# gmlwns2000/sharkshark-4k

Hardware: AMD Instinct MI355X
Metric: upscaled frames/sec at 720p->1440p x2 (whole job) (higher is better)
Workload: dtype f16; 1 GPU; RealESRGAN RRDBNet x2 (23 blocks) 720p->1440p fp16 [BASELINE configs[2]]; io=uint8 NHWC resident in HBM

## Files before the change

sharkshark-4k_amd/csrc/common.h:

```cpp
#pragma once
#include <hip/hip_runtime.h>
#include <hip/hip_fp16.h>
#include <algorithm>
#include <cstdint>
#include <cstdio>
#include <cstdlib>
#include <cstring>
#include <map>
#include <tuple>
#include <set>
#include <string>
#include <vector>
#include <stdexcept>
#include "../../include/ss4k.h"
#ifdef SS4K_DEV
#include "../../include/ss4k_dev.h"
#endif

namespace ss4k {

void set_error(const char* fmt, ...);

struct Error : std::runtime_error {
  int code;
// ... 111 lines not shown
    return lane_stream_;
  }
  static hipEvent_t untimed_event(hipEvent_t& e) {
    if (!e && hipEventCreateWithFlags(&e, hipEventDisableTiming) != hipSuccess) throw ss4k::Error(SS4K_EHIP, "hipEventCreateWithFlags failed");
    return e;
  }
  hipEvent_t lane_fork() { return untimed_event(fork_event); }
  hipEvent_t lane_done() { return untimed_event(done_event); }
  std::set<hipStream_t> lane_checked;
  std::vector<hipStream_t> lane_parked;
  int lane_replaced = 0;
  void lane_check(hipStream_t caller);
#ifdef SS4K_DEV
  int dev_handicap_lane = 0; unsigned dev_handicap_ticks = 0;
  int64_t dev_lane_forks = 0, dev_lane_joins = 0, dev_lane_spins = 0;
  int dev_drop_join = 0;
#endif
  std::vector<ss4k::ProfEvent> prof_sections;
  double prof_section_ms = 0;
  ss4k::ProfEvent prof_get_events() {
    ss4k::ProfEvent pe{};
    if (!prof_pool.empty()) { pe = prof_pool.back(); prof_pool.pop_back(); pe.flops = 0; pe.kind = 0; pe.family = nullptr; return pe; }
    if (hipEventCreate(&pe.a) != hipSuccess || hipEventCreate(&pe.b) != hipSuccess) throw ss4k::Error(SS4K_EHIP, "hipEventCreate failed");
    return pe;
  }
  ss4k::ProfEvent prof_begin(hipStream_t st, int kind) {
    ss4k::ProfEvent pe{};
    if (!prof) return pe;
    pe = prof_get_events(); pe.kind = kind;
    if (hipEventRecord(pe.a, st) != hipSuccess) throw ss4k::Error(SS4K_EHIP, "hipEventRecord failed");
    return pe;
  }
  void prof_end(ss4k::ProfEvent pe, hipStream_t st, double flops) {
    if (!pe.a) return;
    if (hipEventRecord(pe.b, st) != hipSuccess) throw ss4k::Error(SS4K_EHIP, "hipEventRecord failed");
    pe.flops = flops; pe.family = prof_family; prof_family = nullptr; prof_events.push_back(pe);
  }
  const char* zero_page() {
    auto& b = scratch["zero_page"];
    if (!b.ptr) { b.ensure(256); (void)hipMemset(b.ptr, 0, 256); }
    return b.as<char>();
  }
  struct CvAreaTab { std::vector<char> host; ss4k::DevBuf dev; hipEvent_t uploaded = nullptr; int oh = 0, ow = 0; size_t xe = 0, xo = 0, ye = 0, yo = 0; };
  std::map<std::tuple<int, int, double, double>, CvAreaTab> cv_area;
  ss4k::DevBuf& buf(const std::string& name, size_t bytes) {
    auto& b = scratch[name];
    b.ensure(bytes);
#ifdef SS4K_DEV
    b.transient = true;
#endif
    return b;
  }
};

namespace ss4k {

struct ProfScope {
  ss4k_ctx* ctx; hipStream_t st; ProfEvent pe; bool open;
  ProfScope(ss4k_ctx* c, hipStream_t s, int kind) : ctx(c), st(s), pe(c->prof_begin(s, kind)), open(true) {}
  void done(double flops) { if (open) { open = false; ctx->prof_end(pe, st, flops); } }
  ~ProfScope() { if (open && pe.a) ctx->prof_pool.push_back(pe); }
  ProfScope(const ProfScope&) = delete; ProfScope& operator=(const ProfScope&) = delete;
};

enum Act { ACT_NONE = 0, ACT_LRELU = 1, ACT_PRELU = 2, ACT_RELU6 = 3 };
enum Epi {
  EPI_NHWC = 0,
  EPI_NHWC_SUB2 = 1,
  EPI_NHWC_PS2 = 2,
  EPI_NCHW_F32 = 3
};

struct ConvArgs {
  const char* in0; size_t in0_plane_bytes; int in0_plane0, nchunks0;
  const char* in1; size_t in1_plane_bytes; int in1_plane0, nchunks1;
  const char* zero_page;
  int N, H, W;
  int n0;
  int job_n;
  float grid_share;
  int mb_override;
  int wide_rl;
  int wide;
  int no_band;
  int ups2;
  int ups_presum;
  const void* wpk;
  const void* w16;
  const float* bias;
  const float* prelu;
  int prelu_le1;
  int act; float slope;
  float alpha, gamma;
  const char* res1; size_t r1_plane_bytes; int r1_plane0;
  const char* res2; size_t r2_plane_bytes; int r2_plane0;
  int bsvd_resid;
  int epi;
  char* out; size_t out_plane_bytes; int out_plane0;
  int cout_real, cout_pad;
  int tiles_x, tiles_y;
  int reverse;
  double flops;
  int dbg;
  unsigned long long* dbg_buf;
};
inline double conv_plane_span_f16(const ConvArgs& a) { return (double)std::max(a.n0 + a.N, a.job_n) * a.H * a.W * 32.0; }
enum { DBG_NO_STORE = 1, DBG_NO_MMA = 2, DBG_NO_TILE_DMA = 4, DBG_NO_W_DMA = 8, DBG_NO_EPILOGUE = 16, DBG_STAMP = 32 };

void launch_conv3x3(ss4k_ctx* ctx, const ConvArgs& a, int dtype, hipStream_t st);
struct PairArgs {
  const char* in; size_t in_plane_bytes; int in_plane0, planes_a;
  const char* wA; const float* biasA;
  const char* wB; const float* biasB;
  const char* res; size_t res_plane_bytes; int res_plane0;
  const char* zero_page;
  unsigned long long* dbg_buf;
  char* out; size_t out_plane_bytes; int out_plane0;
  int epi;
  int cout_real;
  int n0, N, H, W, bands;
  float grid_share;
  double flops;
};
inline bool conv3x3_pair_eligible(int planes_a, int cout_pad_a, int nchunks_b, int cout_pad_b) {
  return (planes_a == 1 || planes_a == 2) && cout_pad_a == 32 && nchunks_b == 2 && cout_pad_b == 32;
}
void launch_conv3x3_pair(ss4k_ctx* ctx, const PairArgs& a, hipStream_t st);

struct DenseArgs {
  const char* in0; size_t in0_plane_bytes; int in0_plane0, nchunks0;
  const char* in1; size_t in1_plane_bytes; int in1_plane0, nchunks1;
  const char* w1; const float* bias1;
  const char* w2; const float* bias2;
  float slope;
  char* out1; size_t out1_plane_bytes; int out1_plane0;
  char* out2; size_t out2_plane_bytes; int out2_plane0;
  const char* zero_page;
  int n0, N, H, W, tiles_x, tiles_y;
  float grid_share;
  int reverse;
  double flops;
  unsigned long long* dbg_buf;
};
inline bool conv3x3_dense2_eligible(int nchunks_a, int cout_pad_a, int nchunks_b, int cout_pad_b) {
  return cout_pad_a == 32 && cout_pad_b == 32 && nchunks_b == nchunks_a + 2 && nchunks_a >= 2 && nchunks_a % 2 == 0;
}
struct ConvArgs;
bool conv3x3_wide_eligible(const ConvArgs& a, int dtype);
void launch_conv3x3_wide(ss4k_ctx* ctx, const ConvArgs& a, hipStream_t st);
void launch_conv3x3_dense2(ss4k_ctx* ctx, const DenseArgs& a, hipStream_t st);
bool conv3x3_w16_eligible(const ConvArgs& a, int dtype);
void launch_conv3x3_w16(ss4k_ctx* ctx, const ConvArgs& a, hipStream_t st);
bool conv3x3_w16n_eligible(const ConvArgs& a, int dtype);
void launch_conv3x3_w16n(ss4k_ctx* ctx, const ConvArgs& a, hipStream_t st);

inline int conv_cw(int) { return 16; }
inline int cout_pad_of(int cout) { return cout <= 32 ? 32 : (cout + 63) / 64 * 64; }
inline int conv_rec_bytes(int dtype) { return dtype == SS4K_F16 ? 32 : 64; }

struct PackSpec {
  int dtype;
  int cout_real, cin_total;
  std::vector<int> cin_map;
  int nchunks0, nchunks1;
  int ps2;
};
// ... 13 lines not shown
```

sharkshark-4k_amd/csrc/conv_tile.h:

```cpp
#pragma once
#include "common.h"

namespace ss4k {

typedef float f32x16 __attribute__((ext_vector_type(16)));
typedef _Float16 f16x8 __attribute__((ext_vector_type(8)));

constexpr int TW = 32, IN_W = TW + 2;
constexpr uint32_t OOB = 0xFFFFFFFFu;
template <typename T> struct Tr;
template <> struct Tr<__half> { static constexpr int E = 8, KS = 1; };
template <> struct Tr<float> { static constexpr int E = 4, KS = 2; };
constexpr int CW = 16;

template <typename T, int MB, int NW> struct Geo {
  static constexpr int KS = Tr<T>::KS, SPR = 2 * KS, REC = 16 * SPR;
  static constexpr int TH = NW * MB, IN_H = TH + 2, IN_PIX = IN_W * IN_H;
  static constexpr int TILE_SLOTS = IN_PIX * SPR;
  static constexpr int TILE_DMA = (TILE_SLOTS + 63) / 64;
  static constexpr int DMA_PER_WAVE = (TILE_DMA + NW - 1) / NW;
};
template <typename T, int NB, int MB, int NW> constexpr size_t lds_bytes() {
  return (size_t)(2 * Geo<T, MB, NW>::TILE_SLOTS + 2 * 9 * Tr<T>::KS * NB * 64) * 16 + NB * 32 * 2 * 4;
}
template <typename T, int NB, int MB, int NW> constexpr int wgs_per_cu() {
  return NW == 8 ? 1 : (lds_bytes<T, NB, MB, NW>() <= 53 * 1024 ? 3 : lds_bytes<T, NB, MB, NW>() <= 80 * 1024 ? 2 : 1);
}

__device__ __forceinline__ void dma16(const void* gsrc, uint32_t lds_addr_wave_uniform) {
  uint32_t keep;
  asm volatile("s_mov_b32 %0, m0\n\ts_mov_b32 m0, %2\n\ts_nop 0\n\tglobal_load_lds_dwordx4 %1, off\n\ts_mov_b32 m0, %0"
               : "=&s"(keep)
               : "v"(gsrc), "s"(lds_addr_wave_uniform)
               : "memory");
}
__device__ __forceinline__ void dma_wait() { asm volatile("s_waitcnt vmcnt(0)" ::: "memory"); }

template <typename T> __device__ __forceinline__ void load16(const char* p, float* v);
template <> __device__ __forceinline__ void load16<__half>(const char* p, float* v) {
  const uint4 a = *reinterpret_cast<const uint4*>(p), b = *reinterpret_cast<const uint4*>(p + 16);
  const __half* ha = reinterpret_cast<const __half*>(&a);
  const __half* hb = reinterpret_cast<const __half*>(&b);
#pragma unroll
  for (int i = 0; i < 8; ++i) { v[i] = __half2float(ha[i]); v[8 + i] = __half2float(hb[i]); }
}
template <> __device__ __forceinline__ void load16<float>(const char* p, float* v) {
#pragma unroll
  for (int q = 0; q < 4; ++q) {
    const float4 a = *reinterpret_cast<const float4*>(p + 16 * q);
    v[4 * q] = a.x; v[4 * q + 1] = a.y; v[4 * q + 2] = a.z; v[4 * q + 3] = a.w;
  }
}
template <typename T> __device__ __forceinline__ void store16(char* p, const float* v);
template <> __device__ __forceinline__ void store16<__half>(char* p, const float* v) {
  uint4 a, b;
  __half* ha = reinterpret_cast<__half*>(&a);
  __half* hb = reinterpret_cast<__half*>(&b);
#pragma unroll
  for (int i = 0; i < 8; ++i) { ha[i] = __float2half(v[i]); hb[i] = __float2half(v[8 + i]); }
  *reinterpret_cast<uint4*>(p) = a;
  *reinterpret_cast<uint4*>(p + 16) = b;
}
template <> __device__ __forceinline__ void store16<float>(char* p, const float* v) {
#pragma unroll
  for (int q = 0; q < 4; ++q)
    *reinterpret_cast<float4*>(p + 16 * q) = make_float4(v[4 * q], v[4 * q + 1], v[4 * q + 2], v[4 * q + 3]);
}

template <typename T> __device__ __forceinline__ void load8(const char* p, float* v);
template <> __device__ __forceinline__ void load8<__half>(const char* p, float* v) {
  const uint4 a = *reinterpret_cast<const uint4*>(p);
  const __half* ha = reinterpret_cast<const __half*>(&a);
#pragma unroll
  for (int i = 0; i < 8; ++i) v[i] = __half2float(ha[i]);
}
template <> __device__ __forceinline__ void load8<float>(const char* p, float* v) {
#pragma unroll
  for (int q = 0; q < 2; ++q) {
    const float4 a = *reinterpret_cast<const float4*>(p + 16 * q);
    v[4 * q] = a.x; v[4 * q + 1] = a.y; v[4 * q + 2] = a.z; v[4 * q + 3] = a.w;
  }
}
typedef unsigned int u32x4 __attribute__((ext_vector_type(4)));
template <typename T> __device__ __forceinline__ void store8(char* p, const float* v);
template <> __device__ __forceinline__ void store8<__half>(char* p, const float* v) {
  uint4 a;
  __half* ha = reinterpret_cast<__half*>(&a);
#pragma unroll
  for (int i = 0; i < 8; ++i) ha[i] = __float2half(v[i]);
  __builtin_nontemporal_store(*reinterpret_cast<u32x4*>(&a), reinterpret_cast<u32x4*>(p));
}
template <> __device__ __forceinline__ void store8<float>(char* p, const float* v) {
#pragma unroll
  for (int q = 0; q < 2; ++q) {
    const float4 f = make_float4(v[4 * q], v[4 * q + 1], v[4 * q + 2], v[4 * q + 3]);
    __builtin_nontemporal_store(*reinterpret_cast<const u32x4*>(&f), reinterpret_cast<u32x4*>(p + 16 * q));
  }
}

__device__ __forceinline__ void lds_barrier() {
  __builtin_amdgcn_fence(__ATOMIC_RELEASE, "workgroup", "local");
  __builtin_amdgcn_s_barrier();
  __builtin_amdgcn_fence(__ATOMIC_ACQUIRE, "workgroup", "local");
}

template <typename T>
__device__ __forceinline__ f32x16 mma(const uint4& w, const uint4& x, f32x16 acc) {
  if constexpr (sizeof(T) == 2) {
    return __builtin_amdgcn_mfma_f32_32x32x16_f16(*reinterpret_cast<const f16x8*>(&w),
                                                  *reinterpret_cast<const f16x8*>(&x), acc, 0, 0, 0);
  } else {
    const float* wf = reinterpret_cast<const float*>(&w);
    const float* xf = reinterpret_cast<const float*>(&x);
#pragma unroll
    for (int j = 0; j < 4; ++j) acc = __builtin_amdgcn_mfma_f32_32x32x2f32(wf[j], xf[j], acc, 0, 0, 0);
    return acc;
// ... 5 lines not shown
```

sharkshark-4k_amd/csrc/conv_w16.hip:

```cpp
#include "common.h"
#include <cmath>
#include "conv_tile.h"
#include <type_traits>
#include <cstdio>
#include <cstdlib>
#include <vector>

namespace ss4k {
namespace w16 {

typedef float f32x4 __attribute__((ext_vector_type(4)));

constexpr int NW = 4, MB = 8, TH = 16;
constexpr int XH = TH + 2, XW = TW + 2;
constexpr int REC = 32;
constexpr int ROWX = XW * REC;
constexpr int XT_SLOTS = XH * XW * 2;
constexpr int XT_BYTES = XT_SLOTS * 16;
constexpr int XT_DMA = (XT_SLOTS + 63) / 64;
constexpr int DMA_PER_WAVE = (XT_DMA + NW - 1) / NW;
constexpr int WP = 12 * 1024, NWS = 3;
constexpr int NDMA = DMA_PER_WAVE + 3;
constexpr int W_OFF = 2 * XT_BYTES, B_OFF = W_OFF + NWS * WP;
constexpr size_t LDS_BYTES = B_OFF + 2 * 64 * 4;
static_assert(2 * LDS_BYTES <= 160 * 1024, "two workgroups per CU");

__device__ __forceinline__ f32x4 mma16(const uint4& w, const uint4& x, f32x4 acc) {
  return __builtin_amdgcn_mfma_f32_16x16x32_f16(__builtin_bit_cast(f16x8, w), __builtin_bit_cast(f16x8, x), acc, 0, 0, 0);
}

#ifdef SS4K_DEV
template <bool STAMP = false, bool RL = false, bool GEN = false>
#else
template <bool STAMP = false, bool RL = false>
#endif
__global__ __launch_bounds__(64 * NW, 2) void conv3x3_w16_kernel(const ConvArgs a) {
#ifndef SS4K_DEV
  constexpr bool GEN = false;
#endif
  extern __shared__ __attribute__((aligned(16))) char smem[];
  const uint32_t lds0 = (uint32_t)(size_t)(__attribute__((address_space(3))) char*)smem;
  const int tid = threadIdx.x, lane = tid & 63;
  const int wave = __builtin_amdgcn_readfirstlane(tid >> 6);
  const int n16 = lane & 15, kg = lane >> 4;
  const int rgp = wave & 1, jw = wave >> 1;
  const int grp = blockIdx.y;
  const int K = a.nchunks0 + a.nchunks1, NP = K >> 1;
  const int ntiles = a.N * a.tiles_y * a.tiles_x;
  const char* wbase = reinterpret_cast<const char*>(a.w16) + (size_t)grp * NP * (3 * WP);

  unsigned long long ph[6] = {0, 0, 0, 0, 0, 0}, tlast = 0, rt0 = 0, ct0 = 0;
  if constexpr (STAMP) { rt0 = __builtin_amdgcn_s_memrealtime(); ct0 = __builtin_amdgcn_s_memtime(); tlast = ct0; }
  auto stamp = [&](int k) {
    if constexpr (STAMP) {
      unsigned long long t;
      __builtin_amdgcn_sched_barrier(0);
      asm volatile("s_memtime %0\n\ts_waitcnt lgkmcnt(0)" : "=s"(t)::"memory");
      __builtin_amdgcn_sched_barrier(0);
      ph[k] += t - tlast;
      tlast = t;
    }
  };
  const bool banded = (gridDim.x % 8 == 0) && ntiles >= (int)gridDim.x && !a.no_band;
  const int tpx = (ntiles + 7) / 8;
  auto tile_of = [&](int k) -> int {
    if (!banded) {
      const int t = blockIdx.x + k * gridDim.x;
      return t < ntiles ? (a.reverse ? ntiles - 1 - t : t) : -1;
    }
    const int base = (blockIdx.x & 7) * tpx, len = min(tpx, ntiles - base);
    const int j = (blockIdx.x >> 3) + k * (gridDim.x >> 3);
    return j < len ? base + (a.reverse ? len - 1 - j : j) : -1;
  };
  int rdA[2], rdX[2];
#pragma unroll
  for (int hn = 0; hn < 2; ++hn) {
    rdA[hn] = (((rgp * MB) * XW + 16 * hn + n16 + (kg >> 1)) * 2 + (kg & 1)) * 16;
    rdX[hn] = (((rgp * MB) * XW + 16 * hn + n16 + 2) * 2 + (kg & 1)) * 16 + (kg >> 1) * XT_BYTES;
  }

  auto setup_tile = [&](int tile, int& n, int& y0, int& x0) {
    const int tx = tile % a.tiles_x, tyn = tile / a.tiles_x;
    const int ty = tyn % a.tiles_y;
    n = a.n0 + tyn / a.tiles_y; y0 = ty * TH; x0 = tx * TW;
  };
  auto tile_src = [&](int k, int n, int y0, int x0) -> uint32_t {
    const int s = k * 64 + lane;
    const int p = s >> 1, gq = s & 1;
    const int row = p / XW, x = p - row * XW;
    const int iy = y0 - 1 + row, ix = x0 - 1 + x;
    const bool ok = s < XT_SLOTS && iy >= 0 && iy < a.H && ix >= 0 && ix < a.W;
    return ok ? ((uint32_t)(n * a.H + iy) * (uint32_t)a.W + (uint32_t)ix) * REC + (uint32_t)(gq * 16) : OOB;
  };
  auto plane_of = [&](int c) {
    return (c < a.nchunks0) ? a.in0 + (size_t)(a.in0_plane0 + c) * a.in0_plane_bytes
                            : a.in1 + (size_t)(a.in1_plane0 + c - a.nchunks0) * a.in1_plane_bytes;
  };
  const char* pf_plane = nullptr; const char* pf_w = nullptr; int pf_buf = 0, pf_slot = 0, pf_n = 0, pf_y0 = 0, pf_x0 = 0; bool pf_tile = false, pf_wt = false;
  auto dma_op = [&](int idx) {
    if (idx < DMA_PER_WAVE) {
      const int k = wave + NW * idx;
      if (pf_tile && k < XT_DMA) {
        const uint32_t so = tile_src(k, pf_n, pf_y0, pf_x0);
        const char* src = so != OOB ? pf_plane + so : a.zero_page + (lane & 3) * 16;
        const uint32_t dst = __builtin_amdgcn_readfirstlane(lds0 + pf_buf * XT_BYTES + k * 1024);
        if (k * 64 + lane < XT_SLOTS) dma16(src, dst);
      }
    } else if (idx < NDMA) {
      const int k = wave + NW * (idx - DMA_PER_WAVE);
      if (pf_wt) dma16(pf_w + k * 1024 + lane * 16, __builtin_amdgcn_readfirstlane(lds0 + W_OFF + pf_slot * WP + k * 1024));
    }
  };
  auto slot_inc = [](int s) { return s == NWS - 1 ? 0 : s + 1; };
  auto lane_now = [] {
    unsigned z = 0;
    asm volatile("" : "+v"(z));
    return (int)__builtin_amdgcn_mbcnt_hi(~0u, __builtin_amdgcn_mbcnt_lo(~0u, z));
  };

  float* epi_lds = reinterpret_cast<float*>(smem + B_OFF);
  if (tid < 64) {
    const int mbk = tid >> 4, q = (tid >> 2) & 3, i = tid & 3;
    const int vb = grp * 64 + 32 * (mbk >> 1) + 16 * (q >> 1) + 8 * (q & 1) + 4 * (mbk & 1) + i;
    epi_lds[tid] = vb < a.cout_pad ? a.bias[vb] : 0.f;
    const int v = grp * 64 + tid;
    epi_lds[64 + tid] = a.act == ACT_PRELU ? (v < a.cout_pad ? a.prelu[v] : 1.f) : (a.act == ACT_LRELU ? a.slope : (a.act == ACT_RELU6 ? 0.f : 1.f));
  }

  int kt = 0;
  int tile = tile_of(0);
  if (tile < 0) return;
  int n, y0, x0;
  setup_tile(tile, n, y0, x0);
  pf_n = n; pf_y0 = y0; pf_x0 = x0;
  int ws = 0;
  pf_tile = true; pf_plane = plane_of(0); pf_buf = 0; pf_wt = true; pf_w = wbase; pf_slot = 0;
#pragma unroll
  for (int i = 0; i < NDMA; ++i) dma_op(i);
  pf_tile = false; pf_w = wbase + WP; pf_slot = 1;
#pragma unroll
  for (int i = DMA_PER_WAVE; i < NDMA; ++i) dma_op(i);
  dma_wait();
  __syncthreads();
  const int lane16 = lane * 16;
  const int wsub = lane16 + jw * 2048;
  uint4 wf[3][2];
#pragma unroll
  for (int dy = 0; dy < 3; ++dy)
#pragma unroll
    for (int e = 0; e < 2; ++e) wf[dy][e] = *reinterpret_cast<const uint4*>(smem + W_OFF + wsub + (dy * 4 + e) * 1024);

  while (true) {
    f32x4 acc[MB][2][2];
    f32x4 bias4[2];
    {
      const float4* bp = reinterpret_cast<const float4*>(smem + B_OFF + (lane_now() >> 4) * 16 + jw * 128);
      const float4 b0 = bp[0], b1 = bp[4];
      bias4[0] = f32x4{b0.x, b0.y, b0.z, b0.w}; bias4[1] = f32x4{b1.x, b1.y, b1.z, b1.w};
    }
    const int cur_n = n, cur_y0 = y0, cur_x0 = x0;
    const int next_tile = tile_of(kt + 1);
    stamp(0);

    auto period = [&](const int q, auto FIRSTP) {
      const bool last_q = q + 1 == NP;
      auto phase = [&](auto PH, auto FIRST) {
        constexpr int ph = decltype(PH)::value;
        constexpr bool first = decltype(FIRST)::value;
        const int lp2 = 3 * q + ph + 2;
        if (lp2 < 3 * NP) { pf_wt = true; pf_w = wbase + (size_t)lp2 * WP; }
        else if (next_tile >= 0) { pf_wt = true; pf_w = wbase + (size_t)(lp2 - 3 * NP) * WP; }
        else pf_wt = false;
        pf_slot = ws == 0 ? NWS - 1 : ws - 1;
        if constexpr (ph == 0) { pf_tile = true; pf_plane = plane_of(2 * q + 1); pf_buf = 1; }
        else if constexpr (ph == 1) { pf_tile = false; }
        else {
          pf_buf = 0;
          if (!last_q) { pf_tile = true; pf_plane = plane_of(2 * q + 2); }
          else if (next_tile >= 0) { setup_tile(next_tile, n, y0, x0); pf_n = n; pf_y0 = y0; pf_x0 = x0; pf_tile = true; pf_plane = plane_of(0); }
          else pf_tile = false;
        }
        const bool more = !(last_q && ph == 2) || next_tile >= 0;
        const char* tb = smem + (ph == 2 ? XT_BYTES : 0);
        const int* rd = ph == 1 ? rdX : rdA;
        const char* wbn = smem + W_OFF + slot_inc(ws) * WP + wsub;
        uint4 bf[3][2];
        auto bf_load = [&](int t, int hn) { return *reinterpret_cast<const uint4*>(tb + rd[hn] + t * ROWX); };
        bool rl_on = false;
        uint32_t idw[2] = {0u, 0u};
        if constexpr (RL && ph != 1) {
          rl_on = q == jw;
          const int rg = (lane & 15) >> 2, i = lane & 3;
          const bool hit = kg >= 2 && (kg & 1) == (rg & 1) && (rg >> 1) == (ph >> 1);
          const uint32_t hv = hit ? (uint32_t)__half_as_ushort(__float2half(1.f / a.alpha)) << (16 * (i & 1)) : 0u;
          idw[0] = (i >> 1) == 0 ? hv : 0u; idw[1] = (i >> 1) == 1 ? hv : 0u;
        }
#pragma unroll
        for (int t = 0; t < 3; ++t) { bf[t][0] = bf_load(t, 0); bf[t][1] = bf_load(t, 1); }
        int m = 0;
        __builtin_amdgcn_sched_barrier(0);
        __builtin_amdgcn_s_setprio(1);
#pragma unroll
        for (int ir = 0; ir < MB + 2; ++ir) {
#pragma unroll
          for (int dy = 0; dy < 3; ++dy) {
            const int r = ir - dy;
            if (r >= 0 && r < MB) {
#pragma unroll
              for (int hn = 0; hn < 2; ++hn) {
#pragma unroll
                for (int e = 0; e < 2; ++e) acc[r][hn][e] = mma16(wf[dy][e], bf[ir % 3][hn], (first && dy == 0) ? bias4[e] : acc[r][hn][e]);
                if constexpr (RL && ph != 1) {
                  if (dy == 1 && rl_on) {
#pragma unroll
                    for (int e = 0; e < 2; ++e)
                      acc[r][hn][e] = mma16(e == 0 ? make_uint4(idw[0], idw[1], 0u, 0u) : make_uint4(0u, 0u, idw[0], idw[1]), bf[ir % 3][hn], acc[r][hn][e]);
                  }
                }
                const int sl = (m & 1) && m < 10 ? m >> 1 : (m == 13 || m == 17 || m == 21) ? DMA_PER_WAVE + (m - 13) / 4 : -1;
                if (sl >= 0) {
                  __builtin_amdgcn_sched_barrier(0);
                  dma_op(sl);
                  __builtin_amdgcn_sched_barrier(0);
                }
                ++m;
              }
            }
          }
          __builtin_amdgcn_sched_barrier(0);
          if (ir + 3 < MB + 2) { bf[ir % 3][0] = bf_load(ir + 3, 0); bf[ir % 3][1] = bf_load(ir + 3, 1); }
          if (more && ir >= MB - 1) {
            const int dy = ir - (MB - 1);
#pragma unroll
            for (int e = 0; e < 2; ++e) wf[dy][e] = *reinterpret_cast<const uint4*>(wbn + (dy * 4 + e) * 1024);
          }
          __builtin_amdgcn_sched_barrier(0);
        }
        __builtin_amdgcn_s_setprio(0);
        stamp(ph == 1 ? 2 : 1);
        if (more) { dma_wait(); stamp(3); __syncthreads(); stamp(4); }
        ws = slot_inc(ws);
      };
      phase(std::integral_constant<int, 0>{}, FIRSTP);
      phase(std::integral_constant<int, 1>{}, std::false_type{});
      phase(std::integral_constant<int, 2>{}, std::false_type{});
    };
    period(0, std::true_type{});
#pragma unroll 1
    for (int q = 1; q < NP; ++q) period(q, std::false_type{});

    {
      const float alpha = a.alpha, gamma = a.gamma;
      const int le = lane_now();
      const int kge = le >> 4, n16e = le & 15;
      auto load_slopes = [&](float* s) {
        const float4* sp = reinterpret_cast<const float4*>(epi_lds + 64 + 32 * jw + 8 * kge);
        const float4 s0 = sp[0], s1 = sp[1];
        s[0] = s0.x; s[1] = s0.y; s[2] = s0.z; s[3] = s0.w;
        s[4] = s1.x; s[5] = s1.y; s[6] = s1.z; s[7] = s1.w;
      };
      const int opl = grp * 4 + 2 * jw + (kge >> 1);
      const size_t sub = (size_t)(kge & 1) * 16;
      const char* r1p = (a.res1 && !RL) ? a.res1 + (size_t)(a.r1_plane0 + opl) * a.r1_plane_bytes + sub : nullptr;
// ... 281 lines not shown
```

sharkshark-4k_amd/csrc/models.cpp:

```cpp
#include "models.h"
#include <algorithm>
#include <cmath>
#include <cstdlib>
#include <cstring>

namespace ss4k {

static size_t esz(int dtype) { return dtype == SS4K_F16 ? 2 : 4; }
static int pad16(int c) { return (c + 15) / 16 * 16; }


static std::vector<std::pair<int, int>> bsvd_denblock_shapes(const int* chns, int in_ch, int out_ch, int interm) {
  const int c0 = chns[0], c1 = chns[1], c2 = chns[2];
  return {{interm, in_ch}, {c0, interm}, {c1, c0}, {c1, c1}, {c1, c1}, {c2, c1}, {c2, c2}, {c2, c2},
          {c2, c2}, {c2, c2}, {c1 * 4, c2}, {c1, c1}, {c1, c1}, {c0 * 4, c1}, {c0, c0}, {out_ch, c0}};
}

static void validate_desc(const ss4k_model_desc& d);

size_t model_param_count(const ss4k_model_desc& d) {
  try { validate_desc(d); } catch (const Error&) { return 0; }
  switch (d.kind) {
    case SS4K_FSRCNN:
      return 56 * 25 + 56 + 56 + 12 * 56 + 12 + 12 + 4 * (12 * 12 * 9 + 12 + 12) + 56 * 12 + 56 + 56 + 56 * 81 + 1;
// ... 80 lines not shown
  if (a) upload(L.prelu, p.prelu.data(), p.prelu.size() * 4);
  if (use_w16 && use_wide && desc.dtype == SS4K_F16 && p.nb == 2 && p.cout_pad % 64 == 0 && (s.nchunks0 + s.nchunks1) % 2 == 0 && !s.ps2) {
    const std::vector<uint8_t> w6 = pack_conv3x3_w16(s, w, p.cout_pad);
    upload(L.w16, w6.data(), w6.size());
    weight_bytes += w6.size();
  }
  if (use_w16 && desc.dtype == SS4K_F16 && cout <= 4 && (s.nchunks0 + s.nchunks1) % 2 == 0 && !s.ps2) {
    const std::vector<uint8_t> w6 = pack_conv3x3_w16n(s, w);
    upload(L.w16, w6.data(), w6.size());
    weight_bytes += w6.size();
  }
  L.has_prelu = a != nullptr;
  if (a) { L.prelu_le1 = true; for (int c = 0; c < cout; ++c) L.prelu_le1 = L.prelu_le1 && a[c] <= 1.f; }
  L.cout_real = cout; L.cout_pad = p.cout_pad; L.nchunks0 = s.nchunks0; L.nchunks1 = s.nchunks1;
  L.cin_real = 0;
  for (int c : s.cin_map) L.cin_real += c >= 0;
  weight_bytes += p.w.size() + p.bias.size() * 4;
  layers.push_back(std::move(L));
  return (int)layers.size() - 1;
}

PackSpec Model::spec_plain(int cin_real, int ps2) const {
  PackSpec s{}; s.ps2 = ps2; s.nchunks0 = planes_for(cin_real); s.nchunks1 = 0;
  s.cin_map.assign((size_t)s.nchunks0 * cw(), -1);
  for (int j = 0; j < cin_real; ++j) s.cin_map[j] = j;
  return s;
}
PackSpec Model::spec_concat(int c0, int c1) const {
  PackSpec s{}; s.nchunks0 = planes_for(c0); s.nchunks1 = planes_for(c1);
  s.cin_map.assign((size_t)(s.nchunks0 + s.nchunks1) * cw(), -1);
  for (int j = 0; j < c0; ++j) s.cin_map[j] = j;
  for (int j = 0; j < c1; ++j) s.cin_map[(size_t)s.nchunks0 * cw() + j] = c0 + j;
  return s;
}
PackSpec Model::spec_masked(int c) const {
  PackSpec s{}; const int first = (c / 4) / cw();
  s.nchunks0 = planes_for(c) - first; s.nchunks1 = 0;
  s.cin_map.assign((size_t)s.nchunks0 * cw(), -1);
  for (int j = 0; j < s.nchunks0 * cw(); ++j) {
    const int ch = first * cw() + j;
    if (ch >= c / 4 && ch < c) s.cin_map[j] = ch;
  }
  return s;
}

PackSpec Model::spec_shifted(int c) const {
  PackSpec s{}; const int lead = shifted_planes(c);
  s.nchunks0 = lead; s.nchunks1 = planes_for(c) - lead;
  s.cin_map.assign((size_t)planes_for(c) * cw(), -1);
  for (int j = 0; j < c; ++j) s.cin_map[j] = j;
  return s;
}

void Model::build(const float* w, size_t n) {
  validate_desc(desc);
  const int fl = desc.flags;
  SS4K_REQUIRE((fl & ~SS4K_MODEL_FLAGS_ALL) == 0, "desc.flags: unknown SS4K_MODEL_* bit (bits 8, 64, 128, 2048 and 16384 were retired with ABI 3)");
  SS4K_REQUIRE(!((fl & SS4K_MODEL_ONE_CHAIN) && (fl & SS4K_MODEL_TWO_CHAINS)), "desc.flags: ONE_CHAIN and TWO_CHAINS exclude each other");
  SS4K_REQUIRE(!((fl & SS4K_MODEL_TILE_ROWS_16) && (fl & SS4K_MODEL_TILE_ROWS_20)), "desc.flags: TILE_ROWS_16 and TILE_ROWS_20 exclude each other");
  if (fl & SS4K_MODEL_FS_EXACT) fs_exact = true;
  if (fl & SS4K_MODEL_ONE_CHAIN) lanes_mode = 1;
  if (fl & SS4K_MODEL_TWO_CHAINS) lanes_mode = 2;
  if (fl & SS4K_MODEL_TILE_ROWS_16) mb_override = 4;
  if (fl & SS4K_MODEL_TILE_ROWS_20) mb_override = 5;
  if (fl & SS4K_MODEL_NO_PAIR) use_pair = false;
  if (fl & SS4K_MODEL_NO_DENSE) dense_mode = 1;
  if (fl & SS4K_MODEL_HR_F32) hr_f32 = true;
  if (fl & SS4K_MODEL_NO_WIDE) use_wide = false;
  if (fl & SS4K_MODEL_NO_UPS_PRESUM) ups_presum = false;
  if (fl & SS4K_MODEL_NO_W16) use_w16 = false;
  if (!(fl & (SS4K_MODEL_ONE_CHAIN | SS4K_MODEL_TWO_CHAINS)))
    if (const char* e = std::getenv("SS4K_LANES")) lanes_mode = std::max(0, std::min(2, std::atoi(e)));
  if (const char* e = std::getenv("SS4K_FS_EXACT")) fs_exact = fs_exact || e[0] == '1';
#ifdef SS4K_DEV
  if (const char* e = std::getenv("SS4K_NO_FLIP")) flip_walk = !(e[0] == '1');
  if (const char* e = std::getenv("SS4K_SUBBATCH")) sub_batch = std::atoi(e);
  if (const char* e = std::getenv("SS4K_MB")) mb_override = std::atoi(e);
  if (const char* e = std::getenv("SS4K_DENSE_MASK")) dense_mask = std::atoi(e);
  if (const char* e = std::getenv("SS4K_UPS_PRESUM")) ups_presum = e[0] == '1';
  if (const char* e = std::getenv("SS4K_NO_RL")) no_rl = e[0] == '1';
  if (const char* e = std::getenv("SS4K_WIDE_RL")) wide_rl = e[0] == '1';
  if (const char* e = std::getenv("SS4K_WIDE")) use_wide = e[0] == '1';
  if (const char* e = std::getenv("SS4K_W16")) use_w16 = e[0] == '1';
  if (const char* e = std::getenv("SS4K_DENSE_MODE")) dense_mode = std::atoi(e);
  if (const char* e = std::getenv("SS4K_LANE_GRID")) lane_grid_share = (float)std::atof(e);
  if (const char* e = std::getenv("SS4K_FAIL_AT_CONV")) fail_at_conv = std::atoi(e);
#endif
  SS4K_REQUIRE(n == model_param_count(desc), "weight blob size does not match the model description");
  ParamCursor pc{w, n};
  if (desc.kind == SS4K_FSRCNN) {
    weight_bytes = fsrcnn_pack_weights(pc, fs_exact, fs_blob, fsw);
  } else if (desc.kind == SS4K_RRDBNET) {
    const int nf = desc.num_feat, g = desc.num_grow_ch;
    const int cin0 = 3 * (desc.scale == 2 ? 4 : desc.scale == 1 ? 16 : 1);
    add_conv(pc, nf, cin0, spec_plain(cin0), false);
    for (int b = 0; b < desc.num_block; ++b)
      for (int r = 0; r < 3; ++r)
        for (int c = 0; c < 5; ++c) {
          const int co = c < 4 ? g : nf;
          add_conv(pc, co, nf + c * g, c == 0 ? spec_plain(nf) : spec_concat(nf, c * g), false);
        }
    for (int i = 0; i < 4; ++i) add_conv(pc, nf, nf, spec_plain(nf), false);
    add_conv(pc, 3, nf, spec_plain(nf), false);
  } else if (desc.kind == SS4K_SRVGG) {
    const int nf = desc.num_feat;
    add_conv(pc, nf, 3, spec_plain(3), true);
    for (int i = 0; i < desc.num_block; ++i) add_conv(pc, nf, nf, spec_plain(nf), true);
    add_conv(pc, 3 * desc.scale * desc.scale, nf, spec_plain(nf), false);
  } else {
    for (int blk = 0; blk < 2; ++blk) {
      const int ci = blk == 0 ? 4 : desc.bsvd_mid_ch, co = blk == 0 ? desc.bsvd_mid_ch : 3;
      auto shapes = bsvd_denblock_shapes(desc.bsvd_chns, ci, co, desc.bsvd_interm_ch);
      for (size_t i = 0; i < shapes.size(); ++i) {
        const int cout = shapes[i].first, cin = shapes[i].second;
        const bool masked = (i == 3 || i == 4 || i == 6 || i == 7 || i == 8 || i == 9 || i == 11 || i == 12);
        const bool ps2 = (i == 10 || i == 13);
        add_conv(pc, cout, cin, masked ? (desc.bsvd_stream ? spec_shifted(cin) : spec_masked(cin)) : spec_plain(cin, ps2 ? 1 : 0), false);
      }
    }
  }
  SS4K_REQUIRE(pc.pos == n, "internal: weight cursor did not consume the blob");
}

template <typename Args, typename Launch>
void Model::launch_lanes(Args& a, double flops_per_frame, int N, hipStream_t st, Launch launch) {
  if (ctx->prof && !section_open) {
    section = ctx->prof_get_events();
    SS4K_HIP(hipEventRecord(section.a, st));
    section_open = true;
  }
  if (cur_lanes <= 1 || N != cur_n) {
    a.n0 = 0; a.N = N; a.flops = flops_per_frame * N;
    launch(a, st);
    return;
  }
  if (!forked) {
    SS4K_HIP(hipEventRecord(ctx->lane_fork(), st));
    SS4K_HIP(hipStreamWaitEvent(ctx->lane_stream(), ctx->lane_fork(), 0));
    forked = true;
#ifdef SS4K_DEV
    ++ctx->dev_lane_forks;
#endif
  }
#ifdef SS4K_DEV
  if (ctx->dev_handicap_ticks) {
    op_lane_spin(ctx->dev_handicap_ticks, ctx->dev_handicap_lane ? ctx->lane_stream() : st);
    ++ctx->dev_lane_spins;
  }
#endif
  for (int l = 0; l < 2; ++l) {
    a.n0 = N * l / 2; a.N = N * (l + 1) / 2 - a.n0;
    a.grid_share = lane_grid_share;
    a.flops = flops_per_frame * a.N;
    launch(a, l == 0 ? st : ctx->lane_stream());
  }
}

void Model::conv(int li,const Tens& in0, const Tens* in1, int N, int H, int W, const ConvOpts& o, hipStream_t st) {
  if (plan_only) return;
#ifdef SS4K_DEV
  if (fail_at_conv > 0 && ++conv_calls == fail_at_conv) throw Error(SS4K_EINVAL, "injected failure (SS4K_FAIL_AT_CONV)");
#endif
  const ConvLayer& L = layers[li];
  ConvArgs a{};
  a.in0 = in0.p; a.in0_plane_bytes = in0.plane_bytes; a.in0_plane0 = in0.plane0; a.nchunks0 = L.nchunks0;
  if (in1) { a.in1 = in1->p; a.in1_plane_bytes = in1->plane_bytes; a.in1_plane0 = in1->plane0; a.nchunks1 = L.nchunks1; }
  SS4K_REQUIRE((in1 != nullptr) == (L.nchunks1 > 0), "internal: conv segment mismatch");
  a.N = N; a.job_n = N; a.H = H; a.W = W; a.ups2 = o.ups2;
  a.wpk = L.w.ptr; a.w16 = L.w16.ptr; a.bias = L.bias.as<float>(); a.prelu = L.has_prelu ? L.prelu.as<float>() : nullptr; a.prelu_le1 = L.prelu_le1 ? 1 : 0;
  a.act = o.act; a.slope = o.slope; a.alpha = o.alpha; a.gamma = o.gamma;
  if (o.res1) { a.res1 = o.res1->p; a.r1_plane_bytes = o.res1->plane_bytes; a.r1_plane0 = o.res1->plane0; }
  if (o.res2) { a.res2 = o.res2->p; a.r2_plane_bytes = o.res2->plane_bytes; a.r2_plane0 = o.res2->plane0; }
  a.bsvd_resid = o.bsvd_resid;
  a.epi = o.epi; a.out = o.out.p; a.out_plane_bytes = o.out.plane_bytes; a.out_plane0 = o.out.plane0;
  a.cout_real = L.cout_real; a.cout_pad = L.cout_pad;
  a.dbg = dbg; a.dbg_buf = dbg_buf; a.mb_override = mb_override; a.wide = use_wide ? 1 : 0; a.ups_presum = ups_presum ? 1 : 0; a.wide_rl = wide_rl ? 1 : 0;
#ifdef SS4K_DEV
  static const bool no_band = std::getenv("SS4K_NO_BAND") && std::getenv("SS4K_NO_BAND")[0] == '1';
  a.no_band = no_band ? 1 : 0;
#endif
  a.reverse = (flip_walk && (launch_parity ^= 1)) ? 1 : 0;
  const double flops = 2.0 * 9.0 * L.cin_real * L.cout_real * (double)H * W * (o.epi == EPI_NHWC_SUB2 ? 0.25 : 1.0);
  if (use_wide && !no_rl && a.res1 && a.act == ACT_NONE && a.nchunks0 == 4 && a.cout_pad == 64 && !a.ups2 &&
      a.res1 + (size_t)a.r1_plane0 * a.r1_plane_bytes == a.in0 + (size_t)a.in0_plane0 * a.in0_plane_bytes) {
    a.wide_rl = 1;
  }
  launch_lanes(a, flops, N, st, [&](const ConvArgs& la, hipStream_t s) { launch_conv3x3(ctx, la, desc.dtype, s); });
}

bool Model::conv_pair(int li, const Tens& in0, int N, int H, int W, const ConvOpts& o, hipStream_t st) {
  const ConvLayer& A = layers[li]; const ConvLayer& B = layers[li + 1];
  const bool plain_b = o.epi == EPI_NHWC && o.act == ACT_RELU6 && !o.res1 && !o.res2 && !o.bsvd_resid;
  const bool resid_b = (o.epi == EPI_NHWC || o.epi == EPI_NCHW_F32) && o.act == ACT_NONE && o.res1 && !o.res2 && o.bsvd_resid && o.alpha == 1.f;
  if (!use_pair || desc.dtype != SS4K_F16 || dbg || o.ups2 || !(plain_b || resid_b) || A.nchunks1 || B.nchunks1 || A.has_prelu || B.has_prelu ||
      !conv3x3_pair_eligible(A.nchunks0, A.cout_pad, B.nchunks0, B.cout_pad) || (o.epi == EPI_NCHW_F32 && B.cout_real > 8))
    return false;
  if (plan_only) return true;
#ifdef SS4K_DEV
  if (fail_at_conv > 0 && ++conv_calls == fail_at_conv) throw Error(SS4K_EINVAL, "injected failure (SS4K_FAIL_AT_CONV)");
#endif
  PairArgs a{};
  a.in = in0.p; a.in_plane_bytes = in0.plane_bytes; a.in_plane0 = in0.plane0; a.planes_a = A.nchunks0;
  a.wA = reinterpret_cast<const char*>(A.w.ptr); a.biasA = A.bias.as<float>();
  a.wB = reinterpret_cast<const char*>(B.w.ptr); a.biasB = B.bias.as<float>();
  if (o.res1) { a.res = o.res1->p; a.res_plane_bytes = o.res1->plane_bytes; a.res_plane0 = o.res1->plane0; }
  a.out = o.out.p; a.out_plane_bytes = o.out.plane_bytes; a.out_plane0 = o.out.plane0;
  a.epi = plain_b ? 0 : (o.epi == EPI_NHWC ? 1 : 2);
  a.zero_page = ctx->zero_page();
  a.cout_real = B.cout_real;
  a.H = H; a.W = W;
  const double flops = 2.0 * 9.0 * ((double)A.cin_real * A.cout_real + (double)B.cin_real * B.cout_real) * (double)H * W;
  launch_lanes(a, flops, N, st, [&](const PairArgs& la, hipStream_t s) { launch_conv3x3_pair(ctx, la, s); });
  return true;
}

bool Model::conv_dense(int li, const Tens& in0, const Tens* in1, int N, int H, int W, float slope, const Tens& out1, const Tens& out2, hipStream_t st) {
  const ConvLayer& A = layers[li]; const ConvLayer& B = layers[li + 1];
  const int pair_bit = (A.nchunks0 + A.nchunks1) <= 4 ? 1 : 2;
  const bool want = dense_mode != 1;
  if (!want || !(dense_mask & pair_bit) || desc.dtype != SS4K_F16 || dbg || A.has_prelu || B.has_prelu || A.nchunks0 != B.nchunks0 ||
      !conv3x3_dense2_eligible(A.nchunks0 + A.nchunks1, A.cout_pad, B.nchunks0 + B.nchunks1, B.cout_pad) ||
      (double)N * H * W * rec() >= 4294967296.0)
    return false;
  if (plan_only) return true;
#ifdef SS4K_DEV
  if (fail_at_conv > 0 && ++conv_calls == fail_at_conv) throw Error(SS4K_EINVAL, "injected failure (SS4K_FAIL_AT_CONV)");
#endif
  SS4K_REQUIRE((in1 != nullptr) == (A.nchunks1 > 0), "internal: conv segment mismatch");
  DenseArgs a{};
  a.in0 = in0.p; a.in0_plane_bytes = in0.plane_bytes; a.in0_plane0 = in0.plane0; a.nchunks0 = A.nchunks0;
  if (in1) { a.in1 = in1->p; a.in1_plane_bytes = in1->plane_bytes; a.in1_plane0 = in1->plane0; a.nchunks1 = A.nchunks1; }
  a.w1 = A.w.as<char>(); a.bias1 = A.bias.as<float>();
  a.w2 = B.w.as<char>(); a.bias2 = B.bias.as<float>();
  a.slope = slope;
  a.out1 = out1.p; a.out1_plane_bytes = out1.plane_bytes; a.out1_plane0 = out1.plane0;
  a.out2 = out2.p; a.out2_plane_bytes = out2.plane_bytes; a.out2_plane0 = out2.plane0;
  a.H = H; a.W = W;
  a.reverse = (flip_walk && (launch_parity ^= 1)) ? 1 : 0;
  const double flops = 2.0 * 9.0 * ((double)A.cin_real * A.cout_real + (double)B.cin_real * B.cout_real) * (double)H * W;
  launch_lanes(a, flops, N, st, [&](const DenseArgs& la, hipStream_t s) { launch_conv3x3_dense2(ctx, la, s); });
  return true;
}

int Model::tune_step(std::map<std::tuple<int, int, int>, LaneTune>& tab, int n, int h, int w, hipStream_t st) {
  const auto key = std::make_tuple(n, h, w);
  auto it = tab.find(key);
  if (it == tab.end()) {
    if (tab.size() >= LANE_TUNE_MAX) return 1;
    it = tab.emplace(key, LaneTune{}).first;
  }
  LaneTune* t = &it->second;
  if (t->decided) return t->decided;
  const int k = t->calls++;
  if (k < 6) {
    if (k >= 2) {
      auto& ev = t->ev[k - 2];
      SS4K_HIP(hipEventCreate(&ev[0])); SS4K_HIP(hipEventCreate(&ev[1]));
      SS4K_HIP(hipEventRecord(ev[0], st));
      tune_timed = ev[1];
// ... 437 lines not shown
```

sharkshark-4k_amd/csrc/models.h:

```cpp
#pragma once
#include "common.h"
#include "glue.h"
#include "fsrcnn.h"
#include <tuple>

namespace ss4k {

struct Tens { char* p; size_t plane_bytes; int plane0; };

struct ConvLayer {
  DevBuf w, bias, prelu;
  DevBuf w16;
  bool has_prelu = false;
  bool prelu_le1 = false;
  int cout_real = 0, cout_pad = 0, cin_real = 0, nchunks0 = 0, nchunks1 = 0;
};

struct ConvOpts {
  int ups2 = 0;
  int act = ACT_NONE; float slope = 0.f;
  float alpha = 1.f, gamma = 1.f;
  const Tens* res1 = nullptr; const Tens* res2 = nullptr;
  int bsvd_resid = 0;
  int epi = EPI_NHWC;
  Tens out{nullptr, 0, 0};
};

struct ParamCursor {
  const float* base; size_t n, pos = 0;
  const float* take(size_t k) {
    SS4K_REQUIRE(pos + k <= n, "weight blob shorter than the model's state_dict");
    const float* p = base + pos; pos += k; return p;
  }
};
size_t model_param_count(const ss4k_model_desc& d);

struct ForwardOpts {
  double* stats_acc = nullptr;
  bool half_out = false;
  bool u8_in = false;
};

struct Model {
  ss4k_ctx* ctx = nullptr;
  ss4k_model_desc desc{};
  std::vector<ConvLayer> layers;
  std::vector<DevBuf> acts;
  DevBuf fs_blob; FsrcnnWeights fsw{};
  size_t weight_bytes = 0;
  bool flip_walk = true;
  int launch_parity = 0;
  int sub_batch = 0;
  bool plan_only = false;
  std::vector<size_t> plan_bytes;
  size_t workspace_bytes(int n, int h, int w);
  bool hr_f32 = false;
  bool can_u8_in() const { return desc.kind == SS4K_FSRCNN && !fs_exact; }
  bool can_half_out() const {
    return (desc.kind == SS4K_SRVGG || (desc.kind == SS4K_FSRCNN && !fs_exact)) && desc.dtype == SS4K_F16 && !plan_only && !hr_f32;
  }
  int mb_override = 0;
  bool fs_exact = false;
  int lanes_mode = 0;
  float lane_grid_share = 1.f;
  int cur_lanes = 1, cur_n = 0;
  bool forked = false;
  struct LaneTune { int calls = 0, decided = 0; hipEvent_t ev[4][2] = {}; float ms[2] = {}; };
  static constexpr size_t LANE_TUNE_MAX = 64;
  std::map<std::tuple<int, int, int>, LaneTune> lane_tune;
  int tune_step(std::map<std::tuple<int, int, int>, LaneTune>& tab, int n, int h, int w, hipStream_t st);

  hipEvent_t tune_timed = nullptr;
  ProfEvent section{}; bool section_open = false;
  void lanes_begin(int n, int h, int w, hipStream_t st);
  void lanes_join(hipStream_t st, bool end_of_forward);
  int dense_mode = 0;
  bool use_wide = true;
  bool use_w16 = true;
  bool wide_rl = false;
  bool ups_presum = true;
  int dense_mask = 3;
  bool use_pair = true;
  int fail_at_conv = 0, conv_calls = 0, forward_calls = 0;
#ifdef SS4K_DEV
  int dev_mid_joins = 0, dev_drop_at = 0;
  int dev_done_n = 0, dev_done_h = 0, dev_done_w = 0;
#endif
  int dbg = 0;
  unsigned long long* dbg_buf = nullptr;

  void build(const float* w, size_t n);
  bool forward(const float* in, float* out, int n, int h, int w, hipStream_t st, const ForwardOpts& o = {});
  bool forward_impl(const float* in, float* out, int n, int h, int w, hipStream_t st, const ForwardOpts& o);
  void abort_forward(hipStream_t st) noexcept;
  void check_input(int n, int h, int w) const;
  void out_shape(int n, int h, int w, int* oc, int* oh, int* ow) const;
  int in_channels() const;
  bool no_rl = false;
  ~Model() {
    for (auto* tab : {&lane_tune}) for (auto& t : *tab) for (auto& pr : t.second.ev) for (auto e : pr) if (e) (void)hipEventDestroy(e);
  }

  int add_conv(ParamCursor& pc, int cout, int cin_total, PackSpec spec, bool has_prelu_after);
  PackSpec spec_plain(int cin_real, int ps2 = 0) const;
  PackSpec spec_concat(int c0, int c1) const;
  PackSpec spec_masked(int c) const;
  PackSpec spec_shifted(int c) const;
  int shifted_planes(int c) const { return std::min(planes_for(c), (c / 4 + cw() - 1) / cw()); }
  int cw() const { return conv_cw(desc.dtype); }
  int rec() const { return conv_rec_bytes(desc.dtype); }
  int planes_for(int channels) const { return (channels + cw() - 1) / cw(); }
  void conv(int li, const Tens& in0, const Tens* in1, int N, int H, int W, const ConvOpts& o, hipStream_t st);
  bool conv_pair(int li, const Tens& in0, int N, int H, int W, const ConvOpts& o, hipStream_t st);
  bool conv_dense(int li, const Tens& in0, const Tens* in1, int N, int H, int W, float slope, const Tens& out1, const Tens& out2, hipStream_t st);
  Tens act(int idx, size_t pixels, int channels);
  Tens act_planes(int idx, size_t pixels, int planes);
  void pack_in(const float* in, const Tens& dst, int nplanes, int n, int c, int h, int w, int r, hipStream_t st);

 private:
  template <typename Args, typename Launch> void launch_lanes(Args& a, double flops_per_frame, int N, hipStream_t st, Launch launch);
};

}

namespace ss4k {
double bench_conv_layer(ss4k_ctx* ctx, int dtype, int cin0, int cin1, int cout, int n, int h, int w, int flags,
                        int iters, hipStream_t st);
}
struct ss4k_model { ss4k::Model m; };
```

Before: 129.9 frames/s.

## Use scalar-base split DMA for interior halo tiles in w16 conv

For tiles fully inside the image, each tile-plane DMA piece is now issued with a wave-uniform scalar base plus a precomputed per-lane offset that handles the single row-boundary crossing. This replaces the per-lane tile_src bounds check and zero-page fallback. Offsets come from a per-lane table read with v_readlane. The aim is to cut VALU address work and divergence in the prefetch path of the hot RRDB conv kernel. Border tiles keep the general path, and the inline asm that manipulates exec/m0 adds correctness risk.

```diff
diff --git a/sharkshark-4k_amd/csrc/common.h b/sharkshark-4k_amd/csrc/common.h
--- a/sharkshark-4k_amd/csrc/common.h
+++ b/sharkshark-4k_amd/csrc/common.h
@@ -217,6 +217,7 @@
   int mb_override;
   int wide_rl;
   int wide;
+  int halo_scalar;
   int no_band;
   int ups2;
   int ups_presum;
diff --git a/sharkshark-4k_amd/csrc/conv_tile.h b/sharkshark-4k_amd/csrc/conv_tile.h
--- a/sharkshark-4k_amd/csrc/conv_tile.h
+++ b/sharkshark-4k_amd/csrc/conv_tile.h
@@ -32,6 +32,25 @@
   asm volatile("s_mov_b32 %0, m0\n\ts_mov_b32 m0, %2\n\ts_nop 0\n\tglobal_load_lds_dwordx4 %1, off\n\ts_mov_b32 m0, %0"
                : "=&s"(keep)
                : "v"(gsrc), "s"(lds_addr_wave_uniform)
+               : "memory");
+}
+__device__ __forceinline__ void dma16s_split(uint32_t v, uint32_t past_minus_1, uint32_t skip, const void* base_wave_uniform,
+                                             uint32_t lds_addr_wave_uniform) {
+  uint32_t keep, t;
+  asm volatile("v_sub_u32 %1, %3, %2\n\ts_mov_b32 %0, m0\n\tv_lshrrev_b32 %1, 31, %1\n\ts_mov_b32 m0, %6\n\tv_mad_u32_u24 %1, %1, %4, %2\n\t"
+               "s_nop 0\n\tglobal_load_lds_dwordx4 %1, %5\n\ts_mov_b32 m0, %0"
+               : "=&s"(keep), "=&v"(t)
+               : "v"(v), "s"(past_minus_1), "s"(skip), "s"(base_wave_uniform), "s"(lds_addr_wave_uniform)
+               : "memory");
+}
+__device__ __forceinline__ void dma16s_split(uint32_t v, uint32_t past_minus_1, uint32_t skip, const void* base_wave_uniform,
+                                             uint32_t lds_addr_wave_uniform, uint64_t lanes) {
+  uint32_t keep, t;
+  uint64_t ex;
+  asm volatile("v_sub_u32 %1, %4, %3\n\ts_mov_b32 %0, m0\n\tv_lshrrev_b32 %1, 31, %1\n\ts_mov_b32 m0, %7\n\tv_mad_u32_u24 %1, %1, %5, %3\n\t"
+               "s_mov_b64 %2, exec\n\ts_mov_b64 exec, %8\n\tglobal_load_lds_dwordx4 %1, %6\n\ts_mov_b64 exec, %2\n\ts_mov_b32 m0, %0"
+               : "=&s"(keep), "=&v"(t), "=&s"(ex)
+               : "v"(v), "s"(past_minus_1), "s"(skip), "s"(base_wave_uniform), "s"(lds_addr_wave_uniform), "s"(lanes)
                : "memory");
 }
 __device__ __forceinline__ void dma_wait() { asm volatile("s_waitcnt vmcnt(0)" ::: "memory"); }
diff --git a/sharkshark-4k_amd/csrc/conv_w16.hip b/sharkshark-4k_amd/csrc/conv_w16.hip
--- a/sharkshark-4k_amd/csrc/conv_w16.hip
+++ b/sharkshark-4k_amd/csrc/conv_w16.hip
@@ -1,6 +1,7 @@
 #include "common.h"
 #include <cmath>
 #include "conv_tile.h"
+#include "halo_pieces.h"
 #include <type_traits>
 #include <cstdio>
 #include <cstdlib>
@@ -96,11 +97,40 @@
     return (c < a.nchunks0) ? a.in0 + (size_t)(a.in0_plane0 + c) * a.in0_plane_bytes
                             : a.in1 + (size_t)(a.in1_plane0 + c - a.nchunks0) * a.in1_plane_bytes;
   };
-  const char* pf_plane = nullptr; const char* pf_w = nullptr; int pf_buf = 0, pf_slot = 0, pf_n = 0, pf_y0 = 0, pf_x0 = 0; bool pf_tile = false, pf_wt = false;
+  const char* pf_plane = nullptr; const char* pf_w = nullptr; int pf_buf = 0, pf_slot = 0, pf_n = 0, pf_y0 = 0, pf_x0 = 0; bool pf_wt = false;
+  enum { PF_NONE = 0, PF_GENERAL = 1, PF_INSIDE = 2 };
+  int pf_tile = PF_NONE, tile_route = PF_GENERAL; uint32_t pf_t0 = 0;
+  auto aim_tile = [&](int n_, int y0_, int x0_) {
+    pf_n = n_; pf_y0 = y0_; pf_x0 = x0_;
+    tile_route = (a.halo_scalar && a.W < (1 << 19) && halo::W16::interior(a.H, a.W, y0_, x0_)) ? PF_INSIDE : PF_GENERAL;
+    pf_t0 = ((uint32_t)(n_ * a.H + y0_ - 1) * (uint32_t)a.W + (uint32_t)(x0_ - 1)) * REC;
+  };
+  const int lane16 = lane * 16;
+  const int wsub = lane16 + jw * 2048;
+  uint32_t piece_tab;
+  {
+    const int kk = wave + NW * (lane & 7);
+    const uint32_t rel = (uint32_t)(halo::W16::row(kk) * a.W + halo::W16::xs(kk)) * REC - (uint32_t)(jw * 2048);
+    piece_tab = (lane & 8) ? (uint32_t)(halo::W16::split(kk) * 16 + jw * 2048 - 1) : rel;
+  }
   auto dma_op = [&](int idx) {
     if (idx < DMA_PER_WAVE) {
       const int k = wave + NW * idx;
-      if (pf_tile && k < XT_DMA) {
+      static_assert(NW * DMA_PER_WAVE == XT_DMA && halo::W16::PIECES == XT_DMA && halo::W16::SLOTS == XT_SLOTS, "piece geometry");
+      if (pf_tile == PF_INSIDE) {
+        uint32_t rel, past_m1;
+        int l0 = idx;
+        asm volatile("" : "+s"(l0));
+        asm volatile("v_readlane_b32 %0, %2, %3\n\tv_readlane_b32 %1, %2, %4" : "=&s"(rel), "=&s"(past_m1) : "v"(piece_tab), "s"(l0), "s"(l0 | 8));
+        static_assert(DMA_PER_WAVE == 5, "one tab_read per piece of a wave");
+        int wv = wave;
+        asm volatile("" : "+s"(wv));
+        const char* base = pf_plane + (pf_t0 + rel);
+        const uint32_t dst = lds0 + pf_buf * XT_BYTES + (wv + NW * idx) * 1024, skip = (uint32_t)(a.W - XW) * REC;
+        const int kk = wv + NW * idx;
+        if (idx + 1 < DMA_PER_WAVE) dma16s_split((uint32_t)wsub, past_m1, skip, base, dst);
+        else { const int nl = halo::W16::lanes(kk); dma16s_split((uint32_t)wsub, past_m1, skip, base, dst, nl >= 64 ? ~0ull : (1ull << nl) - 1ull); }
+      } else if (pf_tile != PF_NONE) {
         const uint32_t so = tile_src(k, pf_n, pf_y0, pf_x0);
         const char* src = so != OOB ? pf_plane + so : a.zero_page + (lane & 3) * 16;
         const uint32_t dst = __builtin_amdgcn_readfirstlane(lds0 + pf_buf * XT_BYTES + k * 1024);
@@ -132,18 +162,16 @@
   if (tile < 0) return;
   int n, y0, x0;
   setup_tile(tile, n, y0, x0);
-  pf_n = n; pf_y0 = y0; pf_x0 = x0;
+  aim_tile(n, y0, x0);
   int ws = 0;
-  pf_tile = true; pf_plane = plane_of(0); pf_buf = 0; pf_wt = true; pf_w = wbase; pf_slot = 0;
+  pf_tile = tile_route; pf_plane = plane_of(0); pf_buf = 0; pf_wt = true; pf_w = wbase; pf_slot = 0;
 #pragma unroll
   for (int i = 0; i < NDMA; ++i) dma_op(i);
-  pf_tile = false; pf_w = wbase + WP; pf_slot = 1;
+  pf_tile = PF_NONE; pf_w = wbase + WP; pf_slot = 1;
 #pragma unroll
   for (int i = DMA_PER_WAVE; i < NDMA; ++i) dma_op(i);
   dma_wait();
   __syncthreads();
-  const int lane16 = lane * 16;
-  const int wsub = lane16 + jw * 2048;
   uint4 wf[3][2];
 #pragma unroll
   for (int dy = 0; dy < 3; ++dy)
@@ -172,13 +200,13 @@
         else if (next_tile >= 0) { pf_wt = true; pf_w = wbase + (size_t)(lp2 - 3 * NP) * WP; }
         else pf_wt = false;
         pf_slot = ws == 0 ? NWS - 1 : ws - 1;
-        if constexpr (ph == 0) { pf_tile = true; pf_plane = plane_of(2 * q + 1); pf_buf = 1; }
-        else if constexpr (ph == 1) { pf_tile = false; }
+        if constexpr (ph == 0) { pf_tile = tile_route; pf_plane = plane_of(2 * q + 1); pf_buf = 1; }
+        else if constexpr (ph == 1) { pf_tile = PF_NONE; }
         else {
           pf_buf = 0;
-          if (!last_q) { pf_tile = true; pf_plane = plane_of(2 * q + 2); }
-          else if (next_tile >= 0) { setup_tile(next_tile, n, y0, x0); pf_n = n; pf_y0 = y0; pf_x0 = x0; pf_tile = true; pf_plane = plane_of(0); }
-          else pf_tile = false;
+          if (!last_q) { pf_tile = tile_route; pf_plane = plane_of(2 * q + 2); }
+          else if (next_tile >= 0) { setup_tile(next_tile, n, y0, x0); aim_tile(n, y0, x0); pf_tile = tile_route; pf_plane = plane_of(0); }
+          else pf_tile = PF_NONE;
         }
         const bool more = !(last_q && ph == 2) || next_tile >= 0;
         const char* tb = smem + (ph == 2 ? XT_BYTES : 0);
diff --git a/sharkshark-4k_amd/csrc/halo_pieces.h b/sharkshark-4k_amd/csrc/halo_pieces.h
--- /dev/null
+++ b/sharkshark-4k_amd/csrc/halo_pieces.h
@@ -0,0 +1,41 @@
+#pragma once
+
+#ifdef __HIPCC__
+#define SS4K_HALO_HD __host__ __device__ __forceinline__
+#else
+#define SS4K_HALO_HD inline
+#endif
+
+namespace ss4k {
+namespace halo {
+
+template <int XH_, int XW_, int MARGIN_> struct Pieces {
+  static constexpr int XH = XH_, XW = XW_, MARGIN = MARGIN_, REC = 32;
+  static constexpr int SLOTS = XH * XW * 2;
+  static constexpr int PIECES = (SLOTS + 63) / 64;
+  static constexpr int LAST_LANES = SLOTS - 64 * (PIECES - 1);
+  static_assert(XW > 32, "a piece must cross at most one row boundary");
+
+  static SS4K_HALO_HD int row(int j) { return 32 * j / XW; }
+  static SS4K_HALO_HD int xs(int j) { return 32 * j - row(j) * XW; }
+  static SS4K_HALO_HD int split(int j) { const int left = XW - xs(j); return left >= 32 ? 64 : 2 * left; }
+  static SS4K_HALO_HD int lanes(int j) { return j + 1 < PIECES ? 64 : (j + 1 == PIECES ? LAST_LANES : 0); }
+  static SS4K_HALO_HD void slot(int j, int lane, int& r, int& x, int& half) {
+    const bool next = lane >= split(j);
+    r = row(j) + (next ? 1 : 0);
+    x = xs(j) + (lane >> 1) - (next ? XW : 0);
+    half = lane & 1;
+  }
+  static SS4K_HALO_HD unsigned rel(int j, int lane, int W) {
+    return (unsigned)(row(j) * W + xs(j)) * REC + (unsigned)lane * 16u + (lane >= split(j) ? (unsigned)(W - XW) * REC : 0u);
+  }
+  static SS4K_HALO_HD bool interior(int H, int W, int y0, int x0) {
+    return y0 >= MARGIN && y0 - MARGIN + XH <= H && x0 >= MARGIN && x0 - MARGIN + XW <= W;
+  }
+};
+
+typedef Pieces<18, 34, 1> W16;
+typedef Pieces<20, 36, 2> Dense2;
+
+}
+}
diff --git a/sharkshark-4k_amd/csrc/models.cpp b/sharkshark-4k_amd/csrc/models.cpp
--- a/sharkshark-4k_amd/csrc/models.cpp
+++ b/sharkshark-4k_amd/csrc/models.cpp
@@ -186,6 +186,7 @@
   if (const char* e = std::getenv("SS4K_WIDE_RL")) wide_rl = e[0] == '1';
   if (const char* e = std::getenv("SS4K_WIDE")) use_wide = e[0] == '1';
   if (const char* e = std::getenv("SS4K_W16")) use_w16 = e[0] == '1';
+  if (const char* e = std::getenv("SS4K_HALO_GENERAL")) halo_scalar = !(e[0] == '1');
   if (const char* e = std::getenv("SS4K_DENSE_MODE")) dense_mode = std::atoi(e);
   if (const char* e = std::getenv("SS4K_LANE_GRID")) lane_grid_share = (float)std::atof(e);
   if (const char* e = std::getenv("SS4K_FAIL_AT_CONV")) fail_at_conv = std::atoi(e);
@@ -279,6 +280,7 @@
   a.epi = o.epi; a.out = o.out.p; a.out_plane_bytes = o.out.plane_bytes; a.out_plane0 = o.out.plane0;
   a.cout_real = L.cout_real; a.cout_pad = L.cout_pad;
   a.dbg = dbg; a.dbg_buf = dbg_buf; a.mb_override = mb_override; a.wide = use_wide ? 1 : 0; a.ups_presum = ups_presum ? 1 : 0; a.wide_rl = wide_rl ? 1 : 0;
+  a.halo_scalar = halo_scalar ? 1 : 0;
 #ifdef SS4K_DEV
   static const bool no_band = std::getenv("SS4K_NO_BAND") && std::getenv("SS4K_NO_BAND")[0] == '1';
   a.no_band = no_band ? 1 : 0;
diff --git a/sharkshark-4k_amd/csrc/models.h b/sharkshark-4k_amd/csrc/models.h
--- a/sharkshark-4k_amd/csrc/models.h
+++ b/sharkshark-4k_amd/csrc/models.h
@@ -77,6 +77,7 @@
   int dense_mode = 0;
   bool use_wide = true;
   bool use_w16 = true;
+  bool halo_scalar = true;
   bool wide_rl = false;
   bool ups_presum = true;
   int dense_mask = 3;
```

After: 130.5 frames/s, median of 6. About the same (+0.5%).
